# JiahaoPlus/EvoWorld

Hardware: AMD Instinct MI355X
Metric: panoramic frames/sec per clip (576x1024x25f, 25 denoise steps) (higher is better)
Workload: dtype f16

## Files before the change

evoworld_amd/csrc/ff_fused.hip:

```cpp
#include "gemm_common.h"
#include <cstdlib>
#include <type_traits>

namespace {

constexpr int C = 320, HID = 1280, CH = 32, NCH = HID / CH;
constexpr int FF_WM = 4;
constexpr int BM = 128, WAVES_N = 2, NWV = FF_WM * WAVES_N, WROWS = BM / FF_WM, RF = WROWS / 16;
constexpr int KS = C / 32;
constexpr int KT = C / 64;
constexpr int W1_KT = 64 * 128;
constexpr int W1_TILE = KT * W1_KT;
constexpr int W2_TILE = C * CH * 2;
constexpr int HX_TILE = (BM / 16) * 64 * 16;
constexpr int LDS_W1 = 0, LDS_W2 = 2 * W1_TILE, LDS_HX = LDS_W2 + 2 * W2_TILE, LDS_B1 = LDS_HX + 2 * HX_TILE;
constexpr int LDS_SCR = LDS_B1 + 2 * HID * 4;
constexpr int LDS_BYTES = LDS_SCR + 64 * NWV * 8 + 4096;
constexpr int P1 = W1_TILE / 1024 / NWV;
constexpr int P2MAX = (W2_TILE / 1024 + NWV - 1) / NWV;
constexpr int NJ2 = C / 16 / WAVES_N;

struct FfP {
    const f16* x;
    const f16* w1p;
    const f16* b1p;
    const f16* w2p;
    const f16* b2;
    const f16* rowbias;
    const f16* r1;
    const f16* r2;
    const int8_t* r1_lo;
    const int8_t* r2_lo;
    f16* out;
    int8_t* out_lo;
    const f16* zero_page;
    int M, rows_per_group, ld_rowbias, n_tiles;
    float c_acc, c_r1, c_r2;
};

template <bool LO, bool R2>
__global__ __launch_bounds__(64 * NWV, NWV / 4) void ff320_kernel(const FfP p) {
    extern __shared__ __attribute__((aligned(16))) char smem[];
    const int tid = threadIdx.x;
    const int lane = tid & 63;
    const int wave = __builtin_amdgcn_readfirstlane(tid >> 6);
    const unsigned lane16 = (unsigned)(tid & 63) * 16u;
    const int wm = wave >> 1, wn = wave & 1;
    const int frow = lane & 15, fks = lane >> 4, sw = frow & 7;
    if (wave >= NWV / 2) __builtin_amdgcn_s_setprio(1);

    for (int i = tid; i < (2 * W2_TILE + 2 * HX_TILE) / 16; i += 64 * NWV) *(f16x8*)(smem + LDS_W2 + i * 16) = (f16x8){0, 0, 0, 0, 0, 0, 0, 0};
    for (int i = tid; i < 2 * HID / 8; i += 64 * NWV) {
        const f16x8 b = *(const f16x8*)((const char*)p.b1p + i * 16);
#pragma unroll
        for (int e = 0; e < 8; ++e) ((float*)(smem + LDS_B1))[i * 8 + e] = (float)b[e];
    }

    const int G = gridDim.x;
    const int n_my = (p.n_tiles - (int)blockIdx.x + G - 1) / G;
    if (n_my <= 0) return;
    const int CC_total = n_my * NCH;
    if (n_my < (p.n_tiles + G - 1) / G) {
        const int d = (int)(blockIdx.x % 16);
        for (int i = 0; i < d; ++i) __builtin_amdgcn_s_sleep(127);
    }

    auto issue_w1 = [&](int c_mod, int slot) __attribute__((always_inline)) {
        const __amdgpu_buffer_rsrc_t r1d = __builtin_amdgcn_make_buffer_rsrc((void*)((const char*)p.w1p + (size_t)c_mod * W1_TILE), 0, W1_TILE, 0x00020000);
        char* d1 = smem + LDS_W1 + slot * W1_TILE + wave * (P1 * 1024);
#pragma unroll
        for (int k = 0; k < P1; ++k) __builtin_amdgcn_raw_ptr_buffer_load_lds(r1d, (lptr_t)(d1 + k * 1024), 16, (int)lane16, wave * (P1 * 1024) + k * 1024, 0, 0);
    };
    issue_w1(0, 0);
    int cc = 0;
    ew_wait_vm0_lgkm0();
    __syncthreads();
    if (CC_total > 1) issue_w1(1, 1);

    int rd1[2];
#pragma unroll
    for (int h = 0; h < 2; ++h) rd1[h] = (2 * wn * 16 + frow) * 128 + (((h * 4 + fks) ^ sw) << 4);
    const int gq = (0x78 >> (2 * ((frow >> 2) & 3))) & 3;
    const int rd2 = (wn * NJ2 * 16 + frow) * 64 + ((fks ^ gq) << 4);
    const int hx_off = (wm * RF * 64 + lane) * 16;
#define FF_W1F(buf, ks_, j_) (*(const f16x8*)((buf) + ((ks_) >> 1) * W1_KT + (j_) * 2048 + rd1[(ks_) & 1]))

    f16x8 wf[3][2];
    {
        const char* w1b = smem + LDS_W1;
#pragma unroll
        for (int j = 0; j < 2; ++j) { wf[0][j] = FF_W1F(w1b, 0, j); wf[1][j] = FF_W1F(w1b, 1, j); }
    }

    f16x8 xf[RF][KS];
    auto load_x = [&](int tile) __attribute__((always_inline)) {
#pragma unroll
        for (int rf = 0; rf < RF; ++rf) {
            const int m = min(tile * BM + wm * WROWS + rf * 16 + frow, p.M - 1);
            const f16* xp = p.x + (size_t)m * C + fks * 8;
#pragma unroll
            for (int ks = 0; ks < KS; ++ks) xf[rf][ks] = *(const f16x8*)(xp + ks * 32);
        }
    };
    load_x((int)blockIdx.x);
    ew_wait_vm0();

    for (int ti = 0; ti < n_my; ++ti) {
        const int tile = (int)blockIdx.x + ti * G;
        const int m_w0 = tile * BM + wm * WROWS;
        f32x4 acc2[RF][NJ2];
#pragma unroll
        for (int rf = 0; rf < RF; ++rf)
#pragma unroll
            for (int jj = 0; jj < NJ2; ++jj) acc2[rf][jj] = (f32x4){0.f, 0.f, 0.f, 0.f};
        f16x8 hf_old[RF] = {};
        f32x4 acc1p[RF][2] = {};

        auto geglu_rf = [&](const f32x4 (&a)[2], const char* bb, char* dst) __attribute__((always_inline)) {
            const f32x4 va = a[0], gg = a[1];
            const f32x2 o01 = ew_vgelu2((f32x2){va[0], va[1]}, (f32x2){gg[0], gg[1]});
            const f32x2 o23 = ew_vgelu2((f32x2){va[2], va[3]}, (f32x2){gg[2], gg[3]});
            const f16x4 o4 = {(f16)o01[0], (f16)o01[1], (f16)o23[0], (f16)o23[1]};
            *(f16x4*)dst = o4;
        };
        for (int c = 0; c < NCH; ++c, ++cc) {
            const char* w1b = smem + LDS_W1 + (cc & 1) * W1_TILE;
            const char* w1n = smem + LDS_W1 + ((cc + 1) & 1) * W1_TILE;
            const char* w2b = smem + LDS_W2 + ((cc + 1) & 1) * W2_TILE;
            f32x4 acc1[RF][2];
            {
                const char* bc = smem + LDS_B1 + (c * 64 + 2 * wn * 16 + fks * 4) * 4;
                const f32x4 b0 = *(const f32x4*)bc, b1v = *(const f32x4*)(bc + 64);
#pragma unroll
                for (int rf = 0; rf < RF; ++rf) { acc1[rf][0] = b0; acc1[rf][1] = b1v; }
            }
            [[maybe_unused]] const char* bbp = smem + LDS_B1 + ((c > 0 ? c - 1 : 0) * 64 + 2 * wn * 16 + fks * 4) * 2;
            [[maybe_unused]] char* hxp = c > 0 ? smem + LDS_HX + ((cc + 1) & 1) * HX_TILE + hx_off + wn * 8 : smem + LDS_SCR + tid * 8;
#pragma unroll
            for (int ks = 0; ks < KS; ++ks) {
                if (ks + 2 < KS) {
#pragma unroll
                    for (int j = 0; j < 2; ++j) wf[(ks + 2) % 3][j] = FF_W1F(w1b, ks + 2, j);
                }
                ew_pin();
#pragma unroll
                for (int j = 0; j < 2; ++j)
#pragma unroll
                    for (int rf = 0; rf < RF; ++rf)
                        acc1[rf][j] = __builtin_amdgcn_mfma_f32_16x16x32_f16(wf[ks % 3][j], xf[rf][ks], acc1[rf][j], 0, 0, 0);
                static_assert(RF == 2 || RF == 4, "GEGLU slices");
                if constexpr (RF == 2) {
                    if (ks == 1) geglu_rf(acc1p[0], bbp, hxp);
                    if (ks == 5) geglu_rf(acc1p[1], bbp, hxp + 1024);
                } else {
                    if (ks == 1 || ks == 3 || ks == 5 || ks == 7) geglu_rf(acc1p[(ks - 1) / 2], bbp, hxp + ((ks - 1) / 2) * 1024);
                }
                ew_pin();
            }
#pragma unroll
            for (int rf = 0; rf < RF; ++rf) { acc1p[rf][0] = acc1[rf][0]; acc1p[rf][1] = acc1[rf][1]; }
            ew_wait_vm0_lgkm0();
            ew_fence();
            __builtin_amdgcn_s_barrier();
            ew_fence();
            if (c > 0) {
#pragma unroll
                for (int rf = 0; rf < RF; ++rf) hf_old[rf] = *(const f16x8*)(smem + LDS_HX + ((cc + 1) & 1) * HX_TILE + hx_off + rf * 1024);
            }
#pragma unroll
            for (int j = 0; j < 2; ++j) { wf[0][j] = FF_W1F(w1n, 0, j); wf[1][j] = FF_W1F(w1n, 1, j); }
            int c2 = c + 2;
            c2 = c2 >= NCH ? c2 - NCH : c2;
            const __amdgpu_buffer_rsrc_t r1d = __builtin_amdgcn_make_buffer_rsrc((void*)((const char*)p.w1p + (size_t)c2 * W1_TILE), 0, W1_TILE, 0x00020000);
            char* d1 = smem + LDS_W1 + (cc & 1) * W1_TILE + wave * (P1 * 1024);
            const __amdgpu_buffer_rsrc_t r2d = __builtin_amdgcn_make_buffer_rsrc((void*)((const char*)p.w2p + (size_t)c * W2_TILE), 0, W2_TILE, 0x00020000);
            char* d2 = smem + LDS_W2 + (cc & 1) * W2_TILE + wave * 1024;
            ew_pin();
#pragma unroll
            for (int g2 = 0; g2 < 2; ++g2) {
                f16x8 w2f[5];
#pragma unroll
                for (int u = 0; u < 5; ++u) w2f[u] = *(const f16x8*)(w2b + (g2 * 5 + u) * 1024 + rd2);
                ew_pin();
#pragma unroll
                for (int u = 0; u < 5; ++u)
#pragma unroll
                    for (int rf = 0; rf < RF; ++rf)
                        acc2[rf][g2 * 5 + u] = __builtin_amdgcn_mfma_f32_16x16x32_f16(w2f[u], hf_old[rf], acc2[rf][g2 * 5 + u], 0, 0, 0);
                ew_pin();
                constexpr int PER = (P1 + P2MAX + 1) / 2;
#pragma unroll
                for (int k = g2 * PER; k < g2 * PER + PER && k < P1 + P2MAX; ++k) {
                    if (k < P1) __builtin_amdgcn_raw_ptr_buffer_load_lds(r1d, (lptr_t)(d1 + k * 1024), 16, (int)lane16, wave * (P1 * 1024) + k * 1024, 0, 0);
                    else if (wave + NWV * (k - P1) < W2_TILE / 1024)
                        __builtin_amdgcn_raw_ptr_buffer_load_lds(r2d, (lptr_t)(d2 + (k - P1) * NWV * 1024), 16, (int)lane16, wave * 1024 + (k - P1) * NWV * 1024, 0, 0);
                }
                ew_pin();
            }
        }
        {
            {
                const char* bb = smem + LDS_B1 + ((NCH - 1) * 64 + 2 * wn * 16 + fks * 4) * 2;
#pragma unroll
                for (int rf = 0; rf < RF; ++rf) {
                    geglu_rf(acc1p[rf], bb, smem + LDS_HX + ((cc + 1) & 1) * HX_TILE + hx_off + rf * 1024 + wn * 8);
                    acc1p[rf][0] = (f32x4){0.f, 0.f, 0.f, 0.f};
                    acc1p[rf][1] = (f32x4){0.f, 0.f, 0.f, 0.f};
                }
            }
            ew_wait_vm0_lgkm0();
            ew_fence();
            __builtin_amdgcn_s_barrier();
            ew_fence();
            const char* w2b = smem + LDS_W2 + ((cc + 1) & 1) * W2_TILE;
#pragma unroll
            for (int rf = 0; rf < RF; ++rf) hf_old[rf] = *(const f16x8*)(smem + LDS_HX + ((cc + 1) & 1) * HX_TILE + hx_off + rf * 1024);
#pragma unroll
            for (int g2 = 0; g2 < 2; ++g2) {
                f16x8 w2f[5];
#pragma unroll
                for (int u = 0; u < 5; ++u) w2f[u] = *(const f16x8*)(w2b + (g2 * 5 + u) * 1024 + rd2);
#pragma unroll
                for (int u = 0; u < 5; ++u)
#pragma unroll
                    for (int rf = 0; rf < RF; ++rf)
                        acc2[rf][g2 * 5 + u] = __builtin_amdgcn_mfma_f32_16x16x32_f16(w2f[u], hf_old[rf], acc2[rf][g2 * 5 + u], 0, 0, 0);
            }
        }
        {
            const f16* rbp = p.rowbias ? p.rowbias : p.zero_page;
            const f16* r1p = p.r1 ? p.r1 : p.zero_page;
            const f16* r2p = p.r2 ? p.r2 : p.zero_page;
            const int8_t* r1lp = p.r1_lo ? p.r1_lo : (const int8_t*)p.zero_page;
            const int8_t* r2lp = p.r2_lo ? p.r2_lo : (const int8_t*)p.zero_page;
            const int mrb = p.rowbias ? 1 : 0, m1 = p.r1 ? 1 : 0, m2 = p.r2 ? 1 : 0, m1l = p.r1_lo ? 1 : 0, m2l = p.r2_lo ? 1 : 0;
            constexpr int NQ = NJ2 / 2;
            const int n_w0 = wn * (C / WAVES_N) + fks * 8;
#pragma unroll
            for (int rf = 0; rf < RF; ++rf) {
                const int m = m_w0 + rf * 16 + frow;
                const int mc = min(m, p.M - 1);
                const int g = mc / p.rows_per_group;
                f16x8 q1v[NQ], q2v[NQ];
                auto next_x = [&]() __attribute__((always_inline)) { if (rf == RF - 1 && ti + 1 < n_my) load_x(tile + G); };
                u32x2 q1l[NQ], q2l[NQ];
#pragma unroll
                for (int q = 0; q < NQ; ++q) {
                    const int n = n_w0 + q * 32;
                    q1v[q] = *(const f16x8*)(r1p + ((size_t)mc * C + n) * m1);
                    if (LO) q1l[q] = *(const u32x2*)(r1lp + ((size_t)mc * C + n) * m1l);
                    if (R2) {
                        q2v[q] = *(const f16x8*)(r2p + ((size_t)mc * C + n) * m2);
                        if (LO) q2l[q] = *(const u32x2*)(r2lp + ((size_t)mc * C + n) * m2l);
                    }
                }
                next_x();
#pragma unroll
                for (int q = 0; q < NQ; ++q) {
                    const int n = n_w0 + q * 32;
                    const f16x8 bvv = *(const f16x8*)(p.b2 + n);
                    const f16x8 rbv = *(const f16x8*)(rbp + (size_t)(g * p.ld_rowbias + n) * mrb);
                    const f32x4 a0 = acc2[rf][2 * q], a1 = acc2[rf][2 * q + 1];
                    const float vv[8] = {a0[0], a0[1], a0[2], a0[3], a1[0], a1[1], a1[2], a1[3]};
                    f16x8 o;
                    int s8[8];
#pragma unroll
                    for (int e = 0; e < 8; ++e) {
                        float xv = (vv[e] + (float)bvv[e] + (float)rbv[e]) * p.c_acc;
                        if (LO) xv += p.c_r1 * ew_split_dec(q1v[q][e], ew_sbyte(q1l[q][e >> 2], e & 3));
                        else xv += p.c_r1 * (float)q1v[q][e];
                        if (R2) {
                            if (LO) xv += p.c_r2 * ew_split_dec(q2v[q][e], ew_sbyte(q2l[q][e >> 2], e & 3));
                            else xv += p.c_r2 * (float)q2v[q][e];
                        }
                        o[e] = (f16)xv;
                        s8[e] = ew_split_enc(xv, o[e]);
                    }
                    if (m < p.M) {
                        *(f16x8*)(p.out + (size_t)m * C + n) = o;
                        if (LO && p.out_lo)
                            *(u32x2*)(p.out_lo + (size_t)m * C + n) = (u32x2){ew_pack4(s8[0], s8[1], s8[2], s8[3]), ew_pack4(s8[4], s8[5], s8[6], s8[7])};
                    }
                }
            }
        }
        ew_wait_vm0();
    }
    ew_wait_vm0();
}

}


extern "C" ew_status ew_ff_geglu320_f16(const ew_ff_args* a, void* stream) {
    EW_REQUIRE(a != nullptr, "ew_ff_geglu320_f16: null args");
    EW_REQUIRE(a->x && a->w1p && a->b1p && a->w2p && a->b2 && a->out && a->zero_page, "ew_ff_geglu320_f16: null pointer");
    EW_REQUIRE(a->C == C && a->hidden == HID, "ew_ff_geglu320_f16: built for C = 320, hidden = 1280 (got %d, %d)", a->C, a->hidden);
    EW_REQUIRE(a->M > 0 && a->rows_per_group >= 1, "ew_ff_geglu320_f16: bad M / rows_per_group");
    EW_REQUIRE(!a->rowbias || a->ld_rowbias % 8 == 0, "ew_ff_geglu320_f16: ld_rowbias must be a multiple of 8");
    EW_REQUIRE((!a->r1_lo || a->r1) && (!a->r2_lo || a->r2), "ew_ff_geglu320_f16: r1_lo / r2_lo need r1 / r2");
    EW_REQUIRE((long long)a->M * C * 2 < (1LL << 40), "ew_ff_geglu320_f16: M too large");
    FfP p;
    p.x = (const f16*)a->x; p.w1p = (const f16*)a->w1p; p.b1p = (const f16*)a->b1p; p.w2p = (const f16*)a->w2p; p.b2 = (const f16*)a->b2;
    p.rowbias = (const f16*)a->rowbias; p.r1 = (const f16*)a->r1; p.r2 = (const f16*)a->r2;
    p.r1_lo = (const int8_t*)a->r1_lo; p.r2_lo = (const int8_t*)a->r2_lo; p.out = (f16*)a->out; p.out_lo = (int8_t*)a->out_lo;
    p.zero_page = (const f16*)a->zero_page;
    p.M = a->M; p.rows_per_group = a->rows_per_group; p.ld_rowbias = a->rowbias ? a->ld_rowbias : 0;
    p.n_tiles = ew_cdiv(a->M, BM);
    p.c_acc = a->c_acc; p.c_r1 = a->r1 ? a->c_r1 : 0.f; p.c_r2 = a->r2 ? a->c_r2 : 0.f;
    const int ncu = ew_cu_budget();
    const int grid = p.n_tiles < ncu ? p.n_tiles : ncu;
    const bool lo = a->r1_lo || a->r2_lo || a->out_lo;
    const bool r2 = a->r2 != nullptr;
    hipStream_t s = (hipStream_t)stream;
#define FF_LAUNCH(LO_, R2_)                                                                                          \
    do {                                                                                                             \
        static std::atomic<unsigned long long> mask{0};                                                              \
        if (ew_status st = ew_ensure_dynamic_lds((const void*)ff320_kernel<LO_, R2_>, LDS_BYTES, mask)) return st;   \
        hipLaunchKernelGGL((ff320_kernel<LO_, R2_>), dim3(grid), dim3(64 * NWV), LDS_BYTES, s, p);                   \
    } while (0)
    if (lo && r2) FF_LAUNCH(true, true);
    else if (lo) FF_LAUNCH(true, false);
    else if (r2) FF_LAUNCH(false, true);
    else FF_LAUNCH(false, false);
#undef FF_LAUNCH
    return ew_check_launch("ew_ff_geglu320_f16");
}
```

evoworld_amd/csrc/gemm_common.h:

```cpp
#pragma once
#include "common.h"

struct GemmP {
    const f16* a;
    const f16* a2;
    const f16* w;
    const f16* bias;
    const f16* rowbias;
    const f16* r1;
    const f16* r2;
    f16* out;
    const f16* zero_page;
    const int8_t* r1_lo;
    const int8_t* r2_lo;
    int8_t* out_lo;
    int M, N, K;
    int c1, c2, lda, lda2, ld_out, ld_r1, ld_r2, ld_rowbias;
    int mode, n_img, h_in, w_in, h_out, w_out, stride, upsample;
    int tB, tT, tP;
    int conv_shift;
    int rows_per_group, act;
    float c_acc, c_r1, c_r2;
    int tiles_m, tiles_n;
    int band;
    int dbg;
};

struct SkP {
    float* ws;
    unsigned* flags;
    unsigned epoch;
    int tiles, dp_rounds;
};

ew_status ew_conv_small_n_try(const GemmP& p, hipStream_t s, bool* taken);
ew_status ew_gemm3_try(const GemmP& p, hipStream_t s, bool* taken);
ew_status ew_gemm3_try_b256(const GemmP& p, hipStream_t s, bool* taken);
ew_status ew_gemm2_dispatch(const GemmP& p, hipStream_t s);
ew_status ew_gemm1_dispatch(const GemmP& p, hipStream_t s);
ew_status ew_gemm_select_epi(const GemmP& p, int generation, int* epi);
void ew_gemm_note_kernel(const char* fmt, ...);
struct SkInstance { const char* kernel; size_t slot_floats; };
extern const SkInstance ew_gemm3_sk, ew_gemm3_sk_b256;
struct SkWorkspace;
SkWorkspace* ew_sk_workspace(int inst, hipStream_t s);
void ew_sk_begin(int inst, SkWorkspace* w, int mode, int epi, const GemmP& p, SkP* sk);

typedef const __attribute__((address_space(1))) void* gptr_t;
typedef __attribute__((address_space(3))) void* lptr_t;

__device__ __forceinline__ void glds16(const f16* src, char* lds_wave_base) {
    __builtin_amdgcn_global_load_lds((gptr_t)src, (lptr_t)lds_wave_base, 16, 0, 0);
}
```

evoworld_amd/csrc/gemm_dispatch.cpp:

```cpp
#include "gemm_common.h"
#include <mutex>

static int g_gemm_gen = -1;
static int g_gemm_dbg = 0;
static char g_gemm_last_kernel[64] = "";
extern "C" const char* ew_gemm_last_kernel(void) { return g_gemm_last_kernel; }
extern "C" void ew_set_gemm_debug(int d) { g_gemm_dbg = d; }
extern "C" void ew_set_gemm_generation(int gen) { g_gemm_gen = gen; }
extern "C" int ew_get_gemm_generation(void) { return g_gemm_gen < 0 ? (g_gemm_gen = 3) : g_gemm_gen; }
void ew_gemm_note_kernel(const char* fmt, ...) {
    va_list ap;
    va_start(ap, fmt);
    vsnprintf(g_gemm_last_kernel, sizeof(g_gemm_last_kernel), fmt, ap);
    va_end(ap);
}

ew_status ew_gemm_select_epi(const GemmP& p, int generation, int* epi) {
    const bool dense = p.mode == EW_A_DENSE;
    if (p.act == EW_ACT_GEGLU && !dense) { ew_set_error("ew_gemm_f16: GEGLU epilogue is only built for dense mode"); return EW_ERR_UNSUPPORTED; }
    if (p.act == EW_ACT_GEGLU) { *epi = 8; return EW_OK; }
    const int mask = (p.rowbias ? 1 : 0) | (p.r1 ? 2 : 0) | (p.r2 ? 4 : 0);
    if (p.r1_lo || p.r2_lo || p.out_lo) {
        if (generation >= 3 && (mask & 6) == 0) *epi = 16 | 1;
        else if (dense) *epi = (mask & 4) == 0 ? 16 | 3 : 16 | 7;
        else if ((mask & 5) == 0) *epi = 16 | 2;
        else if ((mask & 4) == 0) *epi = 16 | 3;
        else { ew_set_error("ew_gemm_f16: conv modes carry the split residual with row-bias / r1 only (no r2)"); return EW_ERR_UNSUPPORTED; }
        return EW_OK;
    }
    if (mask <= 2 || (dense && mask == 3)) *epi = mask;
    else *epi = dense && (mask == 6 || mask == 4) ? 6 : 7;
    return EW_OK;
}

extern "C" ew_status ew_gemm_f16(const ew_gemm_args* a, void* stream) {
    EW_REQUIRE(a != nullptr, "ew_gemm_f16: null args");
    EW_REQUIRE(a->a && a->w && a->out && a->zero_page, "ew_gemm_f16: null a/w/out/zero_page");
    EW_REQUIRE(a->M > 0 && a->N > 0, "ew_gemm_f16: M,N must be > 0 (M=%d N=%d)", a->M, a->N);
    EW_REQUIRE(a->c1 > 0 && a->c1 % 64 == 0 && a->c2 >= 0 && a->c2 % 64 == 0,
               "ew_gemm_f16: c1,c2 must be multiples of 64 (c1=%d c2=%d)", a->c1, a->c2);
    EW_REQUIRE(a->c2 == 0 || a->a2, "ew_gemm_f16: c2 > 0 needs a2");
    EW_REQUIRE(a->N % 4 == 0 && a->ld_out % 4 == 0, "ew_gemm_f16: N and ld_out must be multiples of 4");
    EW_REQUIRE(a->lda % 8 == 0 && (a->c2 == 0 || a->lda2 % 8 == 0), "ew_gemm_f16: lda must be a multiple of 8");
    EW_REQUIRE(a->rows_per_group >= 1, "ew_gemm_f16: rows_per_group must be >= 1");
    EW_REQUIRE(!a->r1 || a->ld_r1 % 4 == 0, "ew_gemm_f16: ld_r1 must be a multiple of 4");
    EW_REQUIRE(!a->r2 || a->ld_r2 % 4 == 0, "ew_gemm_f16: ld_r2 must be a multiple of 4");
    int taps = 1;
    if (a->mode == EW_A_CONV3X3) {
        taps = 9;
        EW_REQUIRE(a->n_img > 0 && a->h_in > 0 && a->w_in > 0 && a->h_out > 0 && a->w_out > 0 &&
                       (a->stride == 1 || a->stride == 2) && (a->upsample == 0 || a->upsample == 1),
                   "ew_gemm_f16: bad conv3x3 geometry");
        EW_REQUIRE((long long)a->n_img * a->h_out * a->w_out == a->M, "ew_gemm_f16: M != n_img*h_out*w_out");
        EW_REQUIRE(!(a->upsample && a->stride != 1), "ew_gemm_f16: upsample needs stride 1");
        EW_REQUIRE((a->conv_shift == 0 || a->conv_shift == 1) && !(a->conv_shift && a->upsample), "ew_gemm_f16: conv_shift must be 0 or 1 (not with upsample)");
    } else if (a->mode == EW_A_CONVT3) {
        taps = 3;
        EW_REQUIRE(a->tB > 0 && a->tT > 0 && a->tP > 0 && (long long)a->tB * a->tT * a->tP == a->M,
                   "ew_gemm_f16: M != B*T*P");
    } else {
        EW_REQUIRE(a->mode == EW_A_DENSE, "ew_gemm_f16: unknown mode %d", a->mode);
    }
    EW_REQUIRE(a->act == EW_ACT_NONE || a->act == EW_ACT_SILU || a->act == EW_ACT_GEGLU || a->act == EW_ACT_GELU, "ew_gemm_f16: unknown act %d", a->act);
    EW_REQUIRE(!a->rowbias || a->ld_rowbias % 4 == 0, "ew_gemm_f16: ld_rowbias must be a multiple of 4");
    if (a->act == EW_ACT_GEGLU)
        EW_REQUIRE(a->N % 128 == 0 && !a->rowbias && !a->r1 && !a->r2 && !a->out_lo, "ew_gemm_f16: GEGLU needs N %% 128 == 0 and no residuals");
    EW_REQUIRE((!a->r1_lo || a->r1) && (!a->r2_lo || a->r2), "ew_gemm_f16: r1_lo / r2_lo need r1 / r2");
    GemmP p;
    p.a = (const f16*)a->a; p.a2 = (const f16*)a->a2; p.w = (const f16*)a->w; p.bias = (const f16*)a->bias;
    p.rowbias = (const f16*)a->rowbias; p.r1 = (const f16*)a->r1; p.r2 = (const f16*)a->r2; p.out = (f16*)a->out;
    p.zero_page = (const f16*)a->zero_page;
    p.r1_lo = (const int8_t*)a->r1_lo; p.r2_lo = (const int8_t*)a->r2_lo; p.out_lo = (int8_t*)a->out_lo;
    p.conv_shift = a->conv_shift;
    p.M = a->M; p.N = a->N; p.K = taps * (a->c1 + a->c2);
    p.c1 = a->c1; p.c2 = a->c2; p.lda = a->lda; p.lda2 = a->lda2; p.ld_out = a->ld_out; p.ld_r1 = a->ld_r1; p.ld_r2 = a->ld_r2; p.ld_rowbias = a->ld_rowbias;
    p.mode = a->mode; p.n_img = a->n_img; p.h_in = a->h_in; p.w_in = a->w_in; p.h_out = a->h_out; p.w_out = a->w_out;
    p.stride = a->stride; p.upsample = a->upsample; p.tB = a->tB; p.tT = a->tT; p.tP = a->tP;
    p.rows_per_group = a->rows_per_group; p.act = a->act; p.c_acc = a->c_acc; p.c_r1 = a->c_r1; p.c_r2 = a->c_r2;
    p.tiles_m = p.tiles_n = 0;
    p.band = 0;
    p.dbg = g_gemm_dbg;
    hipStream_t s = (hipStream_t)stream;
    const int gen = ew_get_gemm_generation();
    bool taken = false;
    ew_status st = EW_OK;
    if (gen >= 2 && ((st = ew_conv_small_n_try(p, s, &taken)) || taken)) return st;
    if (gen >= 3 && ((st = ew_gemm3_try(p, s, &taken)) || taken)) return st;
    if (gen >= 3 && ((st = ew_gemm3_try_b256(p, s, &taken)) || taken)) return st;
    return gen >= 2 ? ew_gemm2_dispatch(p, s) : ew_gemm1_dispatch(p, s);
}

struct SkDesc { unsigned epoch; int mode, epi, M, N, K; };
constexpr int SK_DESC_RING = 1024, SK_SLOTS = 256, SK_POOL = 64;
struct SkWorkspace { int dev; hipStream_t stream; float* ws; unsigned* flags; unsigned epoch; SkDesc* ring; };
struct SkPool {
    const SkInstance& inst;
    SkWorkspace pool[SK_POOL];
    int used = 0;
    std::mutex mutex;
    SkWorkspace* workspace(hipStream_t stream, bool create) {
        std::lock_guard<std::mutex> lock(mutex);
        int dev = 0;
        if (hipGetDevice(&dev) != hipSuccess) return nullptr;
        for (int i = 0; i < used; ++i)
            if (pool[i].dev == dev && pool[i].stream == stream) return &pool[i];
        if (!create || used == SK_POOL) return nullptr;
        SkWorkspace w{dev, stream, nullptr, nullptr, 0, nullptr};
        if (hipExtMallocWithFlags((void**)&w.ws, SK_SLOTS * inst.slot_floats * sizeof(float), hipDeviceMallocUncached) != hipSuccess) { (void)hipGetLastError(); return nullptr; }
        if (hipExtMallocWithFlags((void**)&w.flags, 2048 * sizeof(unsigned), hipDeviceMallocUncached) != hipSuccess) { (void)hipGetLastError(); (void)hipFree(w.ws); return nullptr; }
        if (hipMemsetAsync(w.flags, 0, 2048 * sizeof(unsigned), stream) != hipSuccess) { (void)hipGetLastError(); (void)hipFree(w.flags); (void)hipFree(w.ws); return nullptr; }
        w.ring = new SkDesc[SK_DESC_RING]();
        pool[used] = w;
        return &pool[used++];
    }
    int status() {
        std::lock_guard<std::mutex> lock(mutex);
        int bad = 0;
        for (int i = 0; i < used; ++i) {
            SkWorkspace* w = &pool[i];
            unsigned word[2] = {0, 0};
            if (hipMemcpy(word, w->flags + 1024, sizeof(word), hipMemcpyDeviceToHost) != hipSuccess) { (void)hipGetLastError(); return -1; }
            if (!word[0]) continue;
            bad = 1;
            const SkDesc d = w->ring[word[1] % SK_DESC_RING];
            if (d.epoch == word[1])
                ew_set_error("stream-K hand-over timed out: %s<%d, %d> M=%d N=%d K=%d (stream-K launch #%u on device %d, stream %p): the output of that launch is invalid",
                         inst.kernel, d.mode, d.epi, d.M, d.N, d.K, word[1], w->dev, (void*)w->stream);
            else
                ew_set_error("stream-K hand-over timed out in stream-K launch #%u on device %d, stream %p (more than %d stream-K launches ago: description no longer kept)",
                         word[1], w->dev, (void*)w->stream, SK_DESC_RING);
        }
        return bad;
    }
};
static SkPool g_sk[2] = {{ew_gemm3_sk}, {ew_gemm3_sk_b256}};

SkWorkspace* ew_sk_workspace(int inst, hipStream_t s) {
    hipStreamCaptureStatus cap = hipStreamCaptureStatusNone;
    if (hipStreamIsCapturing(s, &cap) != hipSuccess) { (void)hipGetLastError(); cap = hipStreamCaptureStatusNone; }
    return g_sk[inst].workspace(s, cap == hipStreamCaptureStatusNone);
}
void ew_sk_begin(int inst, SkWorkspace* w, int mode, int epi, const GemmP& p, SkP* sk) {
    std::lock_guard<std::mutex> lock(g_sk[inst].mutex);
    const unsigned e = ++w->epoch;
    w->ring[e % SK_DESC_RING] = SkDesc{e, mode, epi, p.M, p.N, p.K};
    sk->ws = w->ws; sk->flags = w->flags; sk->epoch = e;
}

extern "C" ew_status ew_gemm_streamk_init(void* stream) {
    const bool a = g_sk[0].workspace((hipStream_t)stream, true) != nullptr;
    const bool b = g_sk[1].workspace((hipStream_t)stream, true) != nullptr;
    if (!a || !b) { ew_set_error("ew_gemm_streamk_init: no stream-K workspace for this (device, stream): allocation failed or all 64 process-wide pool entries are in use; launches on it run the whole-tile schedule"); return EW_ERR_HIP; }
    return EW_OK;
}
extern "C" int ew_gemm_streamk_status(void) {
    const int b = g_sk[1].status();
    const int a = b < 0 ? b : g_sk[0].status();
    return a < 0 ? a : (a | b);
}
```

include/evoworld_hip.h:

```cpp
#ifndef EVOWORLD_HIP_H
#define EVOWORLD_HIP_H
#include <stddef.h>
#include <stdint.h>
#ifdef __cplusplus
extern "C" {
#endif

typedef int ew_status;
#define EW_OK 0
#define EW_ERR_INVALID_ARG (-1)
#define EW_ERR_UNSUPPORTED (-2)
#define EW_ERR_HIP (-3)

#define EW_ABI_VERSION 15
int ew_abi_version(void);
const char* ew_last_error(void);

enum { EW_A_DENSE = 0, EW_A_CONV3X3 = 1, EW_A_CONVT3 = 2 };
enum { EW_ACT_NONE = 0, EW_ACT_SILU = 1, EW_ACT_GEGLU = 2, EW_ACT_GELU = 3  };

typedef struct ew_gemm_args {
    const void* a;
    const void* a2;
    const void* w;
    const void* bias;
    const void* rowbias;
    const void* r1;
    const void* r2;
    void* out;
    const void* zero_page;
    int M, N;
    int c1, c2;
    int lda, lda2;
    int ld_out, ld_r1, ld_r2, ld_rowbias;
    int mode;
    int n_img, h_in, w_in, h_out, w_out, stride, upsample;
    int tB, tT, tP;
    int rows_per_group;
    int act;
    float c_acc, c_r1, c_r2;
    const void* r1_lo;
    const void* r2_lo;
    void* out_lo;
    int conv_shift;
} ew_gemm_args;

ew_status ew_gemm_f16(const ew_gemm_args* args, void* stream);
void ew_set_gemm_generation(int gen);
int ew_get_gemm_generation(void);
const char* ew_gemm_last_kernel(void);
void ew_set_gemm_debug(int flags);
int ew_gemm_streamk_status(void);
ew_status ew_gemm_streamk_init(void* stream);

int ew_set_cu_budget(int n_cus);
int ew_get_cu_budget(void);
void* ew_stream_create_cu_mask(int first_cu, int n_cus);
ew_status ew_stream_destroy(void* stream);

typedef struct ew_ff_args {
    const void* x;
    const void* w1p;
    const void* b1p;
    const void* w2p;
    const void* b2;
    const void* rowbias;
    const void* r1;
    const void* r1_lo;
    const void* r2;
    const void* r2_lo;
    void* out;
    void* out_lo;
    const void* zero_page;
    int M, C, hidden;
    int rows_per_group, ld_rowbias;
    float c_acc, c_r1, c_r2;
} ew_ff_args;
ew_status ew_ff_geglu320_f16(const ew_ff_args* args, void* stream);

size_t ew_groupnorm_workspace_floats(int n_slabs, int rows, int C_tot, int groups);
ew_status ew_groupnorm_stats_f16(const void* x, const void* x_lo, float* ws, int n_slabs, int rows, int C_src, int c_off,
                                 int C_tot, int groups, void* stream);
ew_status ew_groupnorm_finalize(float* ws, int n_slabs, int rows, int C_tot, int groups, void* stream);
ew_status ew_groupnorm_apply_f16(const void* x, const void* x_lo, const float* ws, const void* gamma, const void* beta,
                                 void* y, int n_slabs, int rows, int C_src, int c_off, int C_tot, int groups, float eps,
                                 int silu, void* stream);
ew_status ew_groupnorm_apply_split_f16(const void* x, const void* x_lo, const float* ws, const void* gamma, const void* beta,
                                       void* y, void* y_lo, int ld_y, int n_slabs, int rows, int C_src, int c_off, int C_tot,
                                       int groups, float eps, int silu, void* stream);

ew_status ew_layernorm_f16(const void* x, const void* x_lo, const void* addvec, int rows_per_group, void* x_out,
                           void* x_out_lo, const void* gamma, const void* beta, void* y, int rows, int C, float eps,
                           void* stream);

ew_status ew_attn_spatial_f16(const void* q, const void* k, const void* vt, void* o, int n_seq, int S, int heads,
                              int ld_qk, long long ld_vt, int ld_o, float scale, void* stream);

ew_status ew_attn_spatial_log2_f16(const void* q, const void* k, const void* vt, void* o, int n_seq, int S, int heads,
                                   int ld_qk, long long ld_vt, int ld_o, void* stream);

ew_status ew_attn_temporal_f16(const void* q, const void* k, const void* v, void* o, int B, int T, int S, int heads,
                               int ld, int ld_o, float scale, void* stream);

ew_status ew_nchw_f32_to_nhwc_f16(const float* x, void* y, int N, int C, int H, int W, int ldc, int c_off, float scale,
                                  void* stream);
ew_status ew_nhwc_f16_to_nchw_f32(const void* x, float* y, int N, int C, int H, int W, int ldc, void* stream);
ew_status ew_nchw_f32_to_nhwc_split_f16(const float* x, void* y, int N, int C, int H, int W, int ldc, int c_off, int lo_off,
                                        int dup_off, float scale, void* stream);

ew_status ew_sinusoid_embed_f16(const float* vals, int n_vals, int n_rows, int dim, void* out, void* stream);

ew_status ew_euler_cfg_step(const void* eps, int ld_eps, float* latents, const float* guidance, float sigma,
                            float sigma_next, void* next_in, int cpad, int T, int h, int w, void* stream);
ew_status ew_euler_cfg_step_split(const void* eps, int ld_eps, float* latents, const float* guidance, float sigma,
                                  float sigma_next, void* next_in, int cpad, int lo_off, int dup_off, int T, int h, int w,
                                  void* stream);

ew_status ew_softmax_rows_f16(const void* hi, const void* lo, void* out, long long rows, int cols, long long ld, void* stream);

ew_status ew_time_conv3_f32(const float* x, const float* w, const float* bias, float* y, int B, int T, int C, int HW, void* stream);

ew_status ew_blur_axis_f32(const float* x, const float* kern, int ksize, float* out, long long planes, int H, int W, int axis,
                           void* stream);
ew_status ew_bicubic_resize_f32(const float* x, float* out, int N, int C, int H, int W, int Ho, int Wo, const float* scale,
                                const float* shift, void* stream);
ew_status ew_vit_patchify_f16(const float* x, void* out, int N, int S, int P, int ldk, void* stream);
ew_status ew_attn_small_f16(const void* q, const void* k, const void* v, void* o, int n_seq, int S, int heads, int D, int ld,
                            int ld_o, float scale, void* stream);

ew_status ew_quant_rows_fp8(const void* x, void* q, float* scale, int rows, int K, void* stream);
ew_status ew_gemm_fp8(const void* a, const float* a_scale, const void* w, const float* w_scale, void* out, int M, int N, int K,
                      long long ld_out, float c_acc, void* stream);

ew_status ew_plucker_embed(const float* rays, const float* c2w, float* out, int N, int H, int W, void* stream);

ew_status ew_cube2equi_gather(const uint8_t* faces, int face_channels, const int16_t* lut, uint8_t* pano, int V, int H,
                              int W, int res, void* stream);

ew_status ew_depth_unproject(const float* depth, const float* extr, const float* intr, float* xyz, int S, int H, int W,
                             void* stream);

size_t ew_select_workspace_bytes(void);
ew_status ew_select_kth_f32(const float* x, size_t n, size_t k, void* ws, float* out2, void* stream);
size_t ew_filter_compact_workspace_bytes(size_t n);
ew_status ew_filter_compact(const float* conf, size_t n, float thr, const float* xyz, const float* img, int img_nchw,
                            unsigned hw, float* out_xyz, unsigned* out_rgbx, void* ws, unsigned* total, void* stream);

ew_status ew_splat_cubemap(const float* xyz, size_t npts, const float* w2c, unsigned long long* zbuf, int V, int res,
                           float fx, float fy, float cx, float cy, float z_near, void* stream);
ew_status ew_splat_resolve(const unsigned long long* zbuf, const uint8_t* rgb, int rgb_stride, uint8_t* faces,
                           int face_channels, int V, int res, void* stream);

ew_status ew_equi2pers(const uint8_t* equi, const float* rot, uint8_t* out, int F, int He, int We, int Hp, int Wp,
                       float fov_x_deg, void* stream);

ew_status ew_resize_aa_u8(const uint8_t* src, uint8_t* tmp, uint8_t* dst, const int* kk_h, const int* bounds_h, int ksize_h,
                          const int* kk_v, const int* bounds_v, int ksize_v, int V, int Hi, int Wi, int Ho, int Wo, void* stream);
ew_status ew_u8_hwc_to_f32_chw(const uint8_t* src, float* dst, int V, int H, int W, void* stream);
ew_status ew_f32_chw_to_u8_hwc(const float* src, uint8_t* dst, int V, int H, int W, void* stream);

ew_status ew_pano_yaw_rotate(const void* src, int src_u8, const float* yaw_deg, float* dst, int V, int H, int W, void* stream);

size_t ew_video_metrics_workspace_bytes(int F, int C, int H, int W);
ew_status ew_video_metrics(const void* a, const void* b, int layout, int F, int C, int H, int W, int what, double* sse, double* ssim,
                           void* workspace, void* stream);

ew_status ew_gt_dump_map_u8(const uint8_t* src, uint8_t* dst, size_t n, void* stream);

ew_status ew_equi2cube_u8(const uint8_t* pano, uint8_t* cross, int V, int H, int W, int interpolation, void* stream);

enum { EW_IM2COL_F16_NHWC = 0, EW_IM2COL_U8_HWC = 1, EW_IM2COL_F32_CHW = 2 };
ew_status ew_im2col_f16(const void* src, int src_kind, void* out, int n_img, int h_in, int w_in, int C, int k, int stride, int pad,
                        int h_out, int w_out, int ldk, int relu, int swap_rb, const float* first_affine, void* stream);
ew_status ew_maxpool3s2_relu_f16(const void* src, void* out, int n_img, int h_in, int w_in, int C, int h_out, int w_out, void* stream);
size_t ew_lpips_head_workspace_bytes(int F, int h, int w, int C);
ew_status ew_lpips_head(const void* fa, const void* fb, const float* lin, const double* wy, const double* wx, int F, int h, int w, int C,
                        double n_out, double* acc, void* workspace, void* stream);

#ifdef __cplusplus
}
#endif
#endif
```

Before: 5.373.

## Split last-wave FF tiles across hidden chunks with fp32 workspace reduction

The persistent fused GEGLU feed-forward kernel now handles the partial final wave of row tiles by splitting each remaining tile's hidden dimension across several blocks. Those blocks write fp32 partial sums to a per-stream workspace, and a small tail kernel reduces them and applies the bias/residual epilogue. The aim is to remove the load imbalance where only a few CUs work on the last tiles. The cost is an extra kernel launch, fp32 workspace traffic, and a workspace allocation that is skipped during graph capture unless it was pre-initialized.

```diff
diff --git a/evoworld_amd/csrc/ff_fused.hip b/evoworld_amd/csrc/ff_fused.hip
--- a/evoworld_amd/csrc/ff_fused.hip
+++ b/evoworld_amd/csrc/ff_fused.hip
@@ -1,5 +1,6 @@
 #include "gemm_common.h"
 #include <cstdlib>
+#include <mutex>
 #include <type_traits>
 
 namespace {
@@ -36,7 +37,33 @@
     const f16* zero_page;
     int M, rows_per_group, ld_rowbias, n_tiles;
     float c_acc, c_r1, c_r2;
+    float* ws;
+    int split, tail_tile0, rem;
 };
+
+template <bool LO, bool R2>
+__device__ __forceinline__ void ff_epi8(const FfP& p, const float (&vv)[8], const f16x8& bvv, const f16x8& rbv, const f16x8& q1v, const u32x2& q1l,
+                                        const f16x8& q2v, const u32x2& q2l, int m, int n) {
+    f16x8 o;
+    int s8[8];
+#pragma unroll
+    for (int e = 0; e < 8; ++e) {
+        float xv = (vv[e] + (float)bvv[e] + (float)rbv[e]) * p.c_acc;
+        if (LO) xv += p.c_r1 * ew_split_dec(q1v[e], ew_sbyte(q1l[e >> 2], e & 3));
+        else xv += p.c_r1 * (float)q1v[e];
+        if (R2) {
+            if (LO) xv += p.c_r2 * ew_split_dec(q2v[e], ew_sbyte(q2l[e >> 2], e & 3));
+            else xv += p.c_r2 * (float)q2v[e];
+        }
+        o[e] = (f16)xv;
+        s8[e] = ew_split_enc(xv, o[e]);
+    }
+    if (m < p.M) {
+        *(f16x8*)(p.out + (size_t)m * C + n) = o;
+        if (LO && p.out_lo)
+            *(u32x2*)(p.out_lo + (size_t)m * C + n) = (u32x2){ew_pack4(s8[0], s8[1], s8[2], s8[3]), ew_pack4(s8[4], s8[5], s8[6], s8[7])};
+    }
+}
 
 template <bool LO, bool R2>
 __global__ __launch_bounds__(64 * NWV, NWV / 4) void ff320_kernel(const FfP p) {
@@ -56,11 +83,15 @@
         for (int e = 0; e < 8; ++e) ((float*)(smem + LDS_B1))[i * 8 + e] = (float)b[e];
     }
 
-    const int G = gridDim.x;
-    const int n_my = (p.n_tiles - (int)blockIdx.x + G - 1) / G;
+    const int G = gridDim.x, bid = (int)blockIdx.x;
+    const int n_whole = p.split ? p.tail_tile0 / G : (p.n_tiles - bid + G - 1) / G;
+    const bool has_item = p.split && bid < p.rem * p.split;
+    const int split1 = p.split ? p.split : 1;
+    const int item_tile = p.tail_tile0 + bid / split1, item_nch = NCH / split1, item_c0 = (bid % split1) * item_nch;
+    const int n_my = n_whole + (has_item ? 1 : 0);
     if (n_my <= 0) return;
     const int CC_total = n_my * NCH;
-    if (n_my < (p.n_tiles + G - 1) / G) {
+    if (!p.split && n_my < (p.n_tiles + G - 1) / G) {
         const int d = (int)(blockIdx.x % 16);
         for (int i = 0; i < d; ++i) __builtin_amdgcn_s_sleep(127);
     }
@@ -106,7 +137,11 @@
     ew_wait_vm0();
 
     for (int ti = 0; ti < n_my; ++ti) {
-        const int tile = (int)blockIdx.x + ti * G;
+        const bool part = ti >= n_whole;
+        const int tile = part ? item_tile : bid + ti * G;
+        const int c_lo = part ? item_c0 : 0, c_hi = part ? item_c0 + item_nch : NCH;
+        const int c_nx = has_item && ti + 1 == n_whole ? item_c0 : 0;
+        const int tile_nx = ti + 1 < n_whole ? tile + G : item_tile;
         const int m_w0 = tile * BM + wm * WROWS;
         f32x4 acc2[RF][NJ2];
 #pragma unroll
@@ -123,7 +158,7 @@
             const f16x4 o4 = {(f16)o01[0], (f16)o01[1], (f16)o23[0], (f16)o23[1]};
             *(f16x4*)dst = o4;
         };
-        for (int c = 0; c < NCH; ++c, ++cc) {
+        for (int c = c_lo; c < c_hi; ++c, ++cc) {
             const char* w1b = smem + LDS_W1 + (cc & 1) * W1_TILE;
             const char* w1n = smem + LDS_W1 + ((cc + 1) & 1) * W1_TILE;
             const char* w2b = smem + LDS_W2 + ((cc + 1) & 1) * W2_TILE;
@@ -134,8 +169,8 @@
 #pragma unroll
                 for (int rf = 0; rf < RF; ++rf) { acc1[rf][0] = b0; acc1[rf][1] = b1v; }
             }
-            [[maybe_unused]] const char* bbp = smem + LDS_B1 + ((c > 0 ? c - 1 : 0) * 64 + 2 * wn * 16 + fks * 4) * 2;
-            [[maybe_unused]] char* hxp = c > 0 ? smem + LDS_HX + ((cc + 1) & 1) * HX_TILE + hx_off + wn * 8 : smem + LDS_SCR + tid * 8;
+            [[maybe_unused]] const char* bbp = smem + LDS_B1 + ((c > c_lo ? c - 1 : c_lo) * 64 + 2 * wn * 16 + fks * 4) * 2;
+            [[maybe_unused]] char* hxp = c > c_lo ? smem + LDS_HX + ((cc + 1) & 1) * HX_TILE + hx_off + wn * 8 : smem + LDS_SCR + tid * 8;
 #pragma unroll
             for (int ks = 0; ks < KS; ++ks) {
                 if (ks + 2 < KS) {
@@ -163,13 +198,14 @@
             ew_fence();
             __builtin_amdgcn_s_barrier();
             ew_fence();
-            if (c > 0) {
+            if (c > c_lo) {
 #pragma unroll
                 for (int rf = 0; rf < RF; ++rf) hf_old[rf] = *(const f16x8*)(smem + LDS_HX + ((cc + 1) & 1) * HX_TILE + hx_off + rf * 1024);
             }
 #pragma unroll
             for (int j = 0; j < 2; ++j) { wf[0][j] = FF_W1F(w1n, 0, j); wf[1][j] = FF_W1F(w1n, 1, j); }
             int c2 = c + 2;
+            c2 = c2 >= c_hi ? c2 - c_hi + c_nx : c2;
             c2 = c2 >= NCH ? c2 - NCH : c2;
             const __amdgpu_buffer_rsrc_t r1d = __builtin_amdgcn_make_buffer_rsrc((void*)((const char*)p.w1p + (size_t)c2 * W1_TILE), 0, W1_TILE, 0x00020000);
             char* d1 = smem + LDS_W1 + (cc & 1) * W1_TILE + wave * (P1 * 1024);
@@ -200,7 +236,7 @@
         }
         {
             {
-                const char* bb = smem + LDS_B1 + ((NCH - 1) * 64 + 2 * wn * 16 + fks * 4) * 2;
+                const char* bb = smem + LDS_B1 + ((c_hi - 1) * 64 + 2 * wn * 16 + fks * 4) * 2;
 #pragma unroll
                 for (int rf = 0; rf < RF; ++rf) {
                     geglu_rf(acc1p[rf], bb, smem + LDS_HX + ((cc + 1) & 1) * HX_TILE + hx_off + rf * 1024 + wn * 8);
@@ -227,7 +263,16 @@
                         acc2[rf][g2 * 5 + u] = __builtin_amdgcn_mfma_f32_16x16x32_f16(w2f[u], hf_old[rf], acc2[rf][g2 * 5 + u], 0, 0, 0);
             }
         }
-        {
+        if (part) {
+            float* wsp = p.ws + (size_t)bid * (BM * C) + (wm * WROWS + frow) * C + wn * (C / WAVES_N) + fks * 8;
+#pragma unroll
+            for (int rf = 0; rf < RF; ++rf)
+#pragma unroll
+                for (int q = 0; q < NJ2 / 2; ++q) {
+                    *(f32x4*)(wsp + rf * 16 * C + q * 32) = acc2[rf][2 * q];
+                    *(f32x4*)(wsp + rf * 16 * C + q * 32 + 4) = acc2[rf][2 * q + 1];
+                }
+        } else {
             const f16* rbp = p.rowbias ? p.rowbias : p.zero_page;
             const f16* r1p = p.r1 ? p.r1 : p.zero_page;
             const f16* r2p = p.r2 ? p.r2 : p.zero_page;
@@ -242,7 +287,7 @@
                 const int mc = min(m, p.M - 1);
                 const int g = mc / p.rows_per_group;
                 f16x8 q1v[NQ], q2v[NQ];
-                auto next_x = [&]() __attribute__((always_inline)) { if (rf == RF - 1 && ti + 1 < n_my) load_x(tile + G); };
+                auto next_x = [&]() __attribute__((always_inline)) { if (rf == RF - 1 && ti + 1 < n_my) load_x(tile_nx); };
                 u32x2 q1l[NQ], q2l[NQ];
 #pragma unroll
                 for (int q = 0; q < NQ; ++q) {
@@ -262,25 +307,7 @@
                     const f16x8 rbv = *(const f16x8*)(rbp + (size_t)(g * p.ld_rowbias + n) * mrb);
                     const f32x4 a0 = acc2[rf][2 * q], a1 = acc2[rf][2 * q + 1];
                     const float vv[8] = {a0[0], a0[1], a0[2], a0[3], a1[0], a1[1], a1[2], a1[3]};
-                    f16x8 o;
-                    int s8[8];
-#pragma unroll
-                    for (int e = 0; e < 8; ++e) {
-                        float xv = (vv[e] + (float)bvv[e] + (float)rbv[e]) * p.c_acc;
-                        if (LO) xv += p.c_r1 * ew_split_dec(q1v[q][e], ew_sbyte(q1l[q][e >> 2], e & 3));
-                        else xv += p.c_r1 * (float)q1v[q][e];
-                        if (R2) {
-                            if (LO) xv += p.c_r2 * ew_split_dec(q2v[q][e], ew_sbyte(q2l[q][e >> 2], e & 3));
-                            else xv += p.c_r2 * (float)q2v[q][e];
-                        }
-                        o[e] = (f16)xv;
-                        s8[e] = ew_split_enc(xv, o[e]);
-                    }
-                    if (m < p.M) {
-                        *(f16x8*)(p.out + (size_t)m * C + n) = o;
-                        if (LO && p.out_lo)
-                            *(u32x2*)(p.out_lo + (size_t)m * C + n) = (u32x2){ew_pack4(s8[0], s8[1], s8[2], s8[3]), ew_pack4(s8[4], s8[5], s8[6], s8[7])};
-                    }
+                    ff_epi8<LO, R2>(p, vv, bvv, rbv, q1v[q], q1l[q], q2v[q], q2l[q], m, n);
                 }
             }
         }
@@ -289,7 +316,64 @@
     ew_wait_vm0();
 }
 
-}
+constexpr int TAIL_THREADS = 256;
+template <bool LO, bool R2>
+__global__ __launch_bounds__(TAIL_THREADS) void ff320_tail_kernel(const FfP p) {
+    const int t = (int)blockIdx.x * TAIL_THREADS + (int)threadIdx.x;
+    const int row = t / (C / 8), n = (t % (C / 8)) * 8;
+    const int m = p.tail_tile0 * BM + row;
+    if (row >= p.rem * BM || m >= p.M) return;
+    const float* wp = p.ws + ((size_t)(row / BM) * p.split * BM + row % BM) * C + n;
+    constexpr int NB = 5;
+    f32x4 a0 = {0.f, 0.f, 0.f, 0.f}, a1 = a0;
+    for (int k0 = 0; k0 < p.split; k0 += NB, wp += NB * BM * C) {
+        f32x4 v0[NB], v1[NB];
+#pragma unroll
+        for (int j = 0; j < NB; ++j) {
+            const bool in = k0 + j < p.split;
+            v0[j] = in ? *(const f32x4*)(wp + j * BM * C) : (f32x4){0.f, 0.f, 0.f, 0.f};
+            v1[j] = in ? *(const f32x4*)(wp + j * BM * C + 4) : (f32x4){0.f, 0.f, 0.f, 0.f};
+        }
+#pragma unroll
+        for (int j = 0; j < NB; ++j) { a0 += v0[j]; a1 += v1[j]; }
+    }
+    const float vv[8] = {a0[0], a0[1], a0[2], a0[3], a1[0], a1[1], a1[2], a1[3]};
+    const int g = m / p.rows_per_group;
+    const size_t off = (size_t)m * C + n;
+    const f16x8 z = {0, 0, 0, 0, 0, 0, 0, 0};
+    const f16x8 bvv = *(const f16x8*)(p.b2 + n);
+    const f16x8 rbv = p.rowbias ? *(const f16x8*)(p.rowbias + (size_t)g * p.ld_rowbias + n) : z;
+    const f16x8 q1v = p.r1 ? *(const f16x8*)(p.r1 + off) : z;
+    const f16x8 q2v = R2 && p.r2 ? *(const f16x8*)(p.r2 + off) : z;
+    const u32x2 q1l = LO && p.r1_lo ? *(const u32x2*)(p.r1_lo + off) : (u32x2){0, 0};
+    const u32x2 q2l = LO && R2 && p.r2_lo ? *(const u32x2*)(p.r2_lo + off) : (u32x2){0, 0};
+    ff_epi8<LO, R2>(p, vv, bvv, rbv, q1v, q1l, q2v, q2l, m, n);
+}
+
+constexpr int FFWS_POOL = 64;
+constexpr size_t FFWS_BYTES = (size_t)256 * BM * C * sizeof(float);
+struct FfWorkspace { int dev; hipStream_t stream; float* ws; };
+FfWorkspace g_ffws[FFWS_POOL];
+int g_ffws_used = 0;
+std::mutex g_ffws_mutex;
+float* ff_workspace(hipStream_t stream, bool create) {
+    std::lock_guard<std::mutex> lock(g_ffws_mutex);
+    int dev = 0;
+    if (hipGetDevice(&dev) != hipSuccess) { (void)hipGetLastError(); return nullptr; }
+    for (int i = 0; i < g_ffws_used; ++i)
+        if (g_ffws[i].dev == dev && g_ffws[i].stream == stream) return g_ffws[i].ws;
+    if (!create || g_ffws_used == FFWS_POOL) return nullptr;
+    FfWorkspace w{dev, stream, nullptr};
+    if (hipMalloc((void**)&w.ws, FFWS_BYTES) != hipSuccess) { (void)hipGetLastError(); w.ws = nullptr; }
+    g_ffws[g_ffws_used++] = w;
+    return w.ws;
+}
+std::atomic<int> g_ff_tail_split{1};
+
+}
+
+extern "C" int ew_set_ff_tail_split(int on) { return g_ff_tail_split.exchange(on ? 1 : 0); }
+bool ew_ff_tail_workspace_init(hipStream_t stream) { return ff_workspace(stream, true) != nullptr; }
 
 
 extern "C" ew_status ew_ff_geglu320_f16(const ew_ff_args* a, void* stream) {
@@ -313,11 +397,22 @@
     const bool lo = a->r1_lo || a->r2_lo || a->out_lo;
     const bool r2 = a->r2 != nullptr;
     hipStream_t s = (hipStream_t)stream;
+    const int full = p.n_tiles / ncu, rem = p.n_tiles % ncu;
+    p.ws = nullptr; p.split = 0; p.tail_tile0 = full * ncu; p.rem = rem;
+    if (g_ff_tail_split.load(std::memory_order_relaxed) && full >= 1 && rem > 0 && rem <= ncu / 2) {
+        hipStreamCaptureStatus cap = hipStreamCaptureStatusNone;
+        if (hipStreamIsCapturing(s, &cap) != hipSuccess) { (void)hipGetLastError(); cap = hipStreamCaptureStatusNone; }
+        if ((p.ws = ff_workspace(s, cap == hipStreamCaptureStatusNone)) != nullptr)
+            for (int d = 2; d <= NCH; ++d)
+                if (NCH % d == 0 && rem * d <= ncu) p.split = d;
+    }
 #define FF_LAUNCH(LO_, R2_)                                                                                          \
     do {                                                                                                             \
         static std::atomic<unsigned long long> mask{0};                                                              \
         if (ew_status st = ew_ensure_dynamic_lds((const void*)ff320_kernel<LO_, R2_>, LDS_BYTES, mask)) return st;   \
         hipLaunchKernelGGL((ff320_kernel<LO_, R2_>), dim3(grid), dim3(64 * NWV), LDS_BYTES, s, p);                   \
+        if (p.split)                                                                                                 \
+            hipLaunchKernelGGL((ff320_tail_kernel<LO_, R2_>), dim3(rem * BM * (C / 8) / TAIL_THREADS), dim3(TAIL_THREADS), 0, s, p); \
     } while (0)
     if (lo && r2) FF_LAUNCH(true, true);
     else if (lo) FF_LAUNCH(true, false);
diff --git a/evoworld_amd/csrc/gemm_common.h b/evoworld_amd/csrc/gemm_common.h
--- a/evoworld_amd/csrc/gemm_common.h
+++ b/evoworld_amd/csrc/gemm_common.h
@@ -44,6 +44,7 @@
 extern const SkInstance ew_gemm3_sk, ew_gemm3_sk_b256;
 struct SkWorkspace;
 SkWorkspace* ew_sk_workspace(int inst, hipStream_t s);
+bool ew_ff_tail_workspace_init(hipStream_t s);
 void ew_sk_begin(int inst, SkWorkspace* w, int mode, int epi, const GemmP& p, SkP* sk);
 
 typedef const __attribute__((address_space(1))) void* gptr_t;
diff --git a/evoworld_amd/csrc/gemm_dispatch.cpp b/evoworld_amd/csrc/gemm_dispatch.cpp
--- a/evoworld_amd/csrc/gemm_dispatch.cpp
+++ b/evoworld_amd/csrc/gemm_dispatch.cpp
@@ -150,7 +150,8 @@
 extern "C" ew_status ew_gemm_streamk_init(void* stream) {
     const bool a = g_sk[0].workspace((hipStream_t)stream, true) != nullptr;
     const bool b = g_sk[1].workspace((hipStream_t)stream, true) != nullptr;
-    if (!a || !b) { ew_set_error("ew_gemm_streamk_init: no stream-K workspace for this (device, stream): allocation failed or all 64 process-wide pool entries are in use; launches on it run the whole-tile schedule"); return EW_ERR_HIP; }
+    const bool f = ew_ff_tail_workspace_init((hipStream_t)stream);
+    if (!a || !b || !f) { ew_set_error("ew_gemm_streamk_init: no stream-K%s workspace for this (device, stream): allocation failed or all 64 process-wide pool entries are in use; launches on it run the whole-tile schedule", a && b ? " / feed-forward tail" : ""); return EW_ERR_HIP; }
     return EW_OK;
 }
 extern "C" int ew_gemm_streamk_status(void) {
diff --git a/include/evoworld_hip.h b/include/evoworld_hip.h
--- a/include/evoworld_hip.h
+++ b/include/evoworld_hip.h
@@ -12,7 +12,7 @@
 #define EW_ERR_UNSUPPORTED (-2)
 #define EW_ERR_HIP (-3)
 
-#define EW_ABI_VERSION 15
+#define EW_ABI_VERSION 16
 int ew_abi_version(void);
 const char* ew_last_error(void);
 
@@ -77,6 +77,7 @@
     float c_acc, c_r1, c_r2;
 } ew_ff_args;
 ew_status ew_ff_geglu320_f16(const ew_ff_args* args, void* stream);
+int ew_set_ff_tail_split(int on);
 
 size_t ew_groupnorm_workspace_floats(int n_slabs, int rows, int C_tot, int groups);
 ew_status ew_groupnorm_stats_f16(const void* x, const void* x_lo, float* ws, int n_slabs, int rows, int C_src, int c_off,
```

After: 5.383, median of 6. No clear change (+0.2%).
